# jseppanen/azalea

Hardware: AMD Instinct MI355X
Metric: mcts_sims_per_sec (higher is better)
Workload: dtype f16x3 (fp32 operands split hi+lo f16, fp32 accumulate)

## Files before the change

### azalea_amd/_lib.py

```python
import ctypes as C
import logging
import os
import subprocess

_HERE = os.path.dirname(os.path.abspath(__file__))
LIB_PATH = os.path.join(_HERE, "libazx_hip.so")

MAX_BOARD = 13
CELL_STRIDE = 192
MAX_BATCH = 16
ROW_METRICS = 8


def record_bytes(cells):
    return (16 + 5 * cells + 15) // 16 * 16

EVAL_RESNET, EVAL_UNIFORM, EVAL_UNIFORM_HASH, EVAL_EXTERNAL = 0, 1, 2, 3
FLAG_NO_COMPACT = 1
FLAG_RANDOM_REFLECT = 2
FLAG_TOWER_F16 = 4
EEXTERNAL = -7


class AzxError(RuntimeError):
# ... 74 lines not shown
    "azx_replay_state": (C.c_int, [_vp, _i64p, _i64p, _i64p]),
    "azx_replay_set_state": (C.c_int, [_vp, C.c_int64, C.c_int64]),
    "azx_replay_put": (C.c_int, [_vp, C.c_int64, _i32p, _i32p, _i32p, _f32p, _f32p]),
    "azx_replay_fill": (C.c_int, [_vp, C.c_int64, C.c_int64, _i64p, C.POINTER(PlayStats)]),
    "azx_play_device": (C.c_int, [_vp, C.c_int64, C.c_int64, _i64p, C.POINTER(PlayStats)]),
    "azx_rows_pack": (C.c_int, [_vp, C.c_int64, C.c_int64, _vp]),
    "azx_replay_put_records": (C.c_int, [_vp, C.c_int64, _vp]),
    "azx_replay_put_records_async": (C.c_int, [_vp, C.c_int64, _vp, _vp]),
    "azx_reserve_cus": (C.c_int, [_vp, C.c_int, C.POINTER(C.c_int)]),
    "azx_replay_collate": (C.c_int, [_vp, C.c_int64, _i64p, _vp, _vp, _vp, _vp, _vp, _vp, _i32p]),
    "azx_replay_collate_async": (C.c_int, [_vp, C.c_int64, _i64p, _vp, _vp, _vp, _vp, _vp, _vp, _vp]),
    "azx_replay_set_mover_view": (C.c_int, [_vp, C.c_int]),
    "azx_replay_set_reflect": (C.c_int, [_vp, C.c_int, C.c_uint64]),
    "azx_selftest_arith": (C.c_int, [C.c_int, C.c_int, _f32p, _f32p, _f32p, _f32p, _f32p]),
    "azx_selftest_divide": (C.c_int, [C.c_int, C.c_int, _f32p, _f32p, _f32p, _f32p]),
    "azx_selftest_dirichlet": (C.c_int, [C.c_int, C.c_double, C.c_int, C.c_int, C.c_uint32, _f32p]),
    "azx_debug_choose": (C.c_int, [_vp, _i32p, _f32p]),
    "azx_debug_counters": (C.c_int, [_vp, _u64p]),
    "azx_debug_counters_raw": (C.c_int, [_vp, _u64p, C.c_int64]),
    "azx_kernel_info": (C.c_int, [_vp, C.c_char_p, C.c_int]),
    "azx_debug_set_queue_cap": (C.c_int, [_vp, C.c_int64]),
    "azx_debug_stagger": (C.c_int, [_vp, _i32p]),
    "azx_debug_tower_tiles": (C.c_int, [C.c_int, C.c_char_p, C.POINTER(C.c_uint8), C.POINTER(C.c_uint32), _i32p]),
    "azx_stream": (_vp, [_vp]),
    "azx_set_external_evaluator": (C.c_int, [_vp, _vp, _vp]),
    "azx_match_create": (C.c_int, [_vp, _vp, C.POINTER(_vp)]),
    "azx_match_destroy": (None, [_vp]),
    "azx_match_play": (C.c_int, [_vp, C.c_int64, C.c_int64, C.POINTER(C.c_int8), C.POINTER(C.c_int16),
                                 C.POINTER(C.c_int16), C.POINTER(MatchStats)]),
    "azx_tournament_create": (C.c_int, [C.POINTER(_vp), C.c_int, C.POINTER(_vp)]),
    "azx_tournament_destroy": (None, [_vp]),
    "azx_tournament_play": (C.c_int, [_vp, C.c_int, _i32p, _i32p, C.c_int64, C.c_int64, C.c_int32,
                                      C.POINTER(C.c_int8), C.POINTER(C.c_int16), C.POINTER(C.c_int16),
                                      C.POINTER(MatchStats)]),
    "azx_match_set_harvest": (C.c_int, [_vp, C.c_int]),
    "azx_match_set_first_mover": (C.c_int, [_vp, C.c_int]),
    "azx_match_rows": (C.c_int, [_vp, _i64p]),
    "azx_tournament_set_harvest": (C.c_int, [_vp, C.c_int]),
    "azx_tournament_set_first_mover": (C.c_int, [_vp, C.c_int]),
    "azx_tournament_rows": (C.c_int, [_vp, _i64p]),
    "azx_rows_read": (C.c_int, [_vp, C.c_int64, C.c_int64, _i32p, _i32p, _i32p, _f32p, _f32p, _i64p]),
    "azx_openings_check": (C.c_int, [C.c_int, C.c_int, C.c_int, C.POINTER(C.c_int16), _i32p, _i32p, _i32p]),
    "azx_match_set_openings": (C.c_int, [_vp, C.c_int, C.c_int, C.POINTER(C.c_int16), _i32p]),
    "azx_tournament_set_openings": (C.c_int, [_vp, C.c_int, C.c_int, C.POINTER(C.c_int16), _i32p]),
    "azx_set_playout_cap": (C.c_int, [_vp, C.c_double, C.c_int]),
    "azx_playout_cap_is_full": (C.c_int, [C.c_uint64, C.c_int64, C.c_int, C.c_double]),
# ... 72 lines not shown
```

### azalea_amd/csrc/azx_capi.cpp

```cpp
#include <hip/hip_runtime.h>

#include <algorithm>
#include <cmath>
#include <cstdarg>
#include <cstdio>
#include <cstdlib>
#include <cstring>
#include <map>
#include <mutex>
#include <string>
#include <vector>

#include "../../include/azx.h"
#include "azx_dev.h"
#include "mcts_kernels.h"
#include "net.h"
#include "train.h"
#include "replay_kernels.h"
#include "ext_kernels.h"
#include "match_kernels.h"
#include "playout_cap.h"
#include "resign.h"
#include "tower_tiles.h"

// ... 221 lines not shown
    d.noise_alpha = (float)cfg->noise_alpha;
    d.noise_scale = 0.0;
    d.exploration_depth = cfg->exploration_depth;
    d.temperature = (float)cfg->temperature;
    e->num_batches = cfg->simulations / cfg->search_batch_size + 1;
    e->selects_per_search = e->num_batches * cfg->search_batch_size;
    d.selects_per_search = e->selects_per_search;
    int cap = cfg->nodes_per_game;
    if (cap <= 0) cap = 6 * (e->selects_per_search + 1) * d.ncells + 1024;
    d.cap = cap;

    const size_t G = d.G, bs = d.bs, E = G * bs;
    const size_t pstride = d.ncells + (d.ncells & 1);
    int rc = AZX_OK;
#define A(ptr, count) if (!rc) rc = dev_alloc(e, &ptr, (count))
    A(d.cells, G * d.slots * 64);
    A(d.ghdr, G);
    A(d.thdr, G);
    if (!rc) rc = dev_alloc(e, &d.arena[0], G * (size_t)cap, false);
    if (cfg->flags & AZX_FLAG_NO_COMPACT) d.arena[1] = d.arena[0];
    else if (!rc) rc = dev_alloc(e, &d.arena[1], G * (size_t)cap, false);
    A(d.leaf_node, E); A(d.leaf_len, E); A(d.leaf_eval, E); A(d.leaf_link, E); A(d.leaf_cells, E);
    A(d.leaf_mask, E * 4); A(d.path, E * pstride);
    A(d.ev_board, E * AZX_CELL_STRIDE); A(d.ev_src, E); A(d.ev_flip, E);
    A(d.ev_value, E); A(d.ev_prior, E * AZX_CELL_STRIDE); A(d.n_eval, 4);
    A(d.counters, G * CTR_COUNT); A(d.q_count, 2); A(d.stat_sums, G * 8);
    A(d.resign_ctr, G * RS_COUNT);
    A(d.estop_ctr, G * ES_COUNT);
    A(d.tt_ctr, G * TT_COUNT);
    A(e->g_k, G); A(e->g_legal, G * d.ncells); A(e->g_nn, G);
    A(e->g_cv, G * d.ncells); A(e->g_cw, G * d.ncells); A(e->g_cp, G * d.ncells);
    A(e->g_rv, G); A(e->g_rw, G); A(e->g_sv, G);
    A(e->moveids_dev, G); A(e->slots_dev, G); A(e->nmoves_dev, G);
#undef A
    if (rc) { azx_destroy(e); return rc; }
    if (cfg->evaluator == AZX_EVAL_RESNET) {
        rc = azx_net_create(&e->net, d.N, cfg->num_blocks, cfg->base_chans, (int)E,
                            (cfg->flags & AZX_FLAG_TOWER_F16) ? 1 : 0, e->stream);
        if (rc) { g_err = azx_net_error(); azx_destroy(e); return rc; }
    }
    {
        float *gt = nullptr;
        rc = dev_alloc(e, &gt, AZX_GAMMA_TAB_FLOATS);
        if (rc) { azx_destroy(e); return rc; }
        std::vector<float> tab(AZX_GAMMA_TAB_FLOATS, 0.0f);
        if (cfg->noise_alpha > 0.0) azx_gamma_table(cfg->noise_alpha, tab.data());
        if (hipMemcpyAsync(gt, tab.data(), tab.size() * sizeof(float), hipMemcpyHostToDevice, e->stream) != hipSuccess ||
// ... 184 lines not shown
    return (int)text.size();
}

extern "C" int azx_debug_stagger(azx_engine *e, int32_t *out4) {
    if (!e || !out4) return fail(AZX_EINVAL, "null argument");
    ENGINE_GUARD(e);
    memset(out4, 0, 4 * sizeof(int32_t));
    if (!e->stagger_ctr) return AZX_OK;
    HIPCHECK(hipMemcpyAsync(out4, e->stagger_ctr, 4 * sizeof(int32_t), hipMemcpyDeviceToHost, e->stream));
    HIPCHECK(hipStreamSynchronize(e->stream));
    return AZX_OK;
}

extern "C" int azx_debug_tower_tiles(int board_size, const char *map, uint8_t *rows256, uint32_t *skip4, int32_t *light_slot) {
    if (!map || !rows256 || !skip4 || !light_slot) return fail(AZX_EINVAL, "null argument");
    if (board_size < 2 || board_size * board_size > 121)
        return fail(AZX_EINVAL, "tower tiles: board size %d outside the fused tower's 2..11", board_size);
    if (strcmp(map, "edge") && strcmp(map, "rows")) return fail(AZX_EINVAL, "tower tiles: map '%s' is neither edge nor rows", map);
    AzxTowerTiles t;
    azx_tower_tiles_build(board_size, !strcmp(map, "edge"), &t);
    memcpy(rows256, t.row, sizeof t.row);
    for (int w = 0; w < 4; ++w) skip4[w] = t.skip[w];
    *light_slot = AZX_TOWER_LIGHT_SLOT;
    return t.edge;
}

extern "C" int azx_debug_set_queue_cap(azx_engine *e, int64_t rows) {
    if (!e || rows < 0) return fail(AZX_EINVAL, "bad argument");
    e->dbg_qcap = rows;
    return AZX_OK;
}

static int check_net_range(azx_engine *e) {
    if (!e->net) return AZX_OK;
    int rc = azx_net_check_range(e->net, e->stream);
    if (rc) g_err = azx_net_error();
    return rc;
}

extern "C" int azx_debug_weights(azx_engine *e, int which, void *out, int64_t cap, int64_t *nbytes, char *name, int name_cap) {
    if (!e) return fail(AZX_EINVAL, "null engine");
    ENGINE_GUARD(e);
    if (!e->net) return fail(AZX_ESTATE, "engine was not created with AZX_EVAL_RESNET");
    int rc = azx_net_debug_weights(e->net, which, out, cap, nbytes, name, name_cap);
    if (rc) g_err = azx_net_error();
    return rc;
// ... 2279 lines not shown
```

### azalea_amd/csrc/net.h

```cpp
#pragma once
#include <hip/hip_runtime.h>
#include <stdint.h>

#include "azx_dev.h"

struct AzxNet;

int azx_net_create(AzxNet **out, int N, int blocks, int chans, int max_evals, int tower_f16, hipStream_t st);
bool azx_net_has_fused_tower(int N, int blocks, int chans);
bool azx_net_has_f16_tower(int N, int blocks, int chans);
void azx_net_destroy(AzxNet *net);
void azx_net_set_stream(AzxNet *net, hipStream_t st, const uint32_t *mask, int words);
const char *azx_net_error();
int azx_net_set_weights(AzxNet *net, int n, const char *const *names, const void *const *ptrs,
                        const int64_t *counts, int on_device);
bool azx_net_ready(const AzxNet *net);
int azx_net_check_range(AzxNet *net, hipStream_t st);
int azx_net_debug_weights(AzxNet *net, int which, void *out, int64_t cap, int64_t *nbytes, char *name, int name_cap);
const char *azx_net_kernel_info(const AzxNet *net);
void azx_net_eval(AzxNet *net, const DevEngine &d, hipStream_t st);
bool azx_net_rows_splittable(const AzxNet *net);
void azx_net_eval_rows(AzxNet *net, const DevEngine &d, int row0, int max_n, hipStream_t st);
constexpr int AZX_NET_ROW_ALIGN = 16;
void azx_net_eval_rows_behind(AzxNet *net, const DevEngine &d, int row0, int first, int max_n, int32_t *ctr, hipStream_t st);
int azx_net_forward_host(AzxNet *net, int B, int K, const int32_t *boards,
                         const int32_t *legal_moves, float *value, float *logprob, hipStream_t st);

int azx_net_wide_train_conv(int N, int C, const unsigned short *w16, const unsigned short *in, float *out32, int n_boards,
                            const float *unscale, float2 *stat, hipStream_t st);
int azx_net_wide_train_conv_bwd(int N, int C, const unsigned short *w16, const unsigned short *in, float *g_out, int n_boards,
                                const float *unscale, float2 *pgsum, const unsigned char *mask, const float *raw, const float *skip,
                                const double *sums, float invN, unsigned int *gmax, hipStream_t st);
```

### azalea_amd/csrc/net_kernels.hip

```cpp
#include "net_priv.h"
#include "tower_tiles.h"

#ifndef AZX_NET_ABLATE
#define AZX_NET_ABLATE 0
#endif
#ifndef AZX_SAT_TRACK
#define AZX_SAT_TRACK 1
#endif

#include <cmath>
#include <cstdio>
#include <cstdlib>
#include <cstring>
#include <map>
#include <string>
#include <type_traits>
#include <utility>
#include <vector>

typedef float f32x16 __attribute__((ext_vector_type(16)));

static thread_local std::string g_net_err;
const char *azx_net_error() { return g_net_err.c_str(); }

// ... 168 lines not shown
#define WT_FLUSH if (lane == 0) { for (int r_ = 0; r_ < 7; ++r_) atomicAdd(&g_wide_stamp[r_], nt_acc[r_]); atomicAdd(&g_wide_stamp[7], 1ull); \
    atomicAdd(&g_wide_stamp[8], __builtin_amdgcn_s_memrealtime() - nt_rt0); }
#else
#define NT_DECL
#define NT_MARK(r)
#define NT_FLUSH
#define WT_FLUSH
#endif

#ifndef F16X3_BPB
#define F16X3_BPB 2
#endif
#ifndef AZX_S16_FENCE
#define AZX_S16_FENCE 1
#endif
typedef float f32x4 __attribute__((ext_vector_type(4)));

__global__ __launch_bounds__(F16X3_BPB * 128, 2) void k_tower_f16x3_s16(NetDev P, const uint8_t *__restrict__ ev_board,
                                                                        const int32_t *__restrict__ n_eval_ptr,
                                                                        int n_eval_host, float *__restrict__ act_out,
                                                                        float *__restrict__ hfeat) {
    constexpr int C = 64, ROWB = 272, MT = 4, NT = 4;
    extern __shared__ __align__(16) unsigned char smem[];
    const int n_eval = n_eval_ptr ? *n_eval_ptr : n_eval_host;
    const int e0 = blockIdx.x * F16X3_BPB;
    if (e0 >= n_eval) return;
    const int tid = threadIdx.x, lane = tid & 63, wave = __builtin_amdgcn_readfirstlane(tid >> 6);
    NT_DECL
    const int wb = wave >> 1, wh = wave & 1;
    const int N = P.N, ncells = P.ncells;
    const int e = e0 + wb;
    const bool live = e < n_eval;
    const int board_b = 128 * ROWB;
    const int zero_off = 0;
    const int x_off = 2 * ROWB + wb * board_b;
    unsigned char *X = smem + x_off;
    const int li = lane & 15, lh = lane >> 4;
    const int lrow = li < 8 ? li ^ 4 : li;
    const int lchunk = 128 * (lh & 1) + 16 * (lh >> 1);

    constexpr int LT = AZX_TOWER_LIGHT_SLOT;
    static_assert(LT == MT - 1, "the k-loop skips the lagging last tile");
    const uint8_t *tmap = P.tile_map + 64 * wave + lrow;
    const uint32_t skip = __builtin_amdgcn_readfirstlane((uint32_t)(P.tile_skip >> (9 * wave)) & 0x1ffu);
    unsigned long long tapok = 0ull;
    int rbase[MT], cell0_[MT];
#pragma unroll
    for (int m = 0; m < MT; ++m) {
        const int L = tmap[16 * m];
        const int r = L & 127;
        const int ry = r / N, rx = r - ry * N;
        cell0_[m] = r < ncells ? 2 * ROWB + (L >> 7) * board_b + 121 * ROWB + ry * (N + 2) + rx : -1;
        rbase[m] = 2 * ROWB + L * ROWB + lchunk;
#pragma unroll
        for (int tap = 0; tap < 9; ++tap) {
            const int yy = ry + tap / 3 - 1, xx = rx + tap % 3 - 1;
            if (r < ncells && yy >= 0 && yy < N && xx >= 0 && xx < N) tapok |= 1ull << (tap * 4 + m);
        }
    }
    uint32_t tapok_lo = (uint32_t)tapok, tapok_hi = (uint32_t)(tapok >> 32);
    auto act_offset = [&](int tap, int m) -> int {
        const int delta = ((tap / 3 - 1) * N + (tap % 3 - 1)) * ROWB;
        const uint32_t word = tap < 8 ? tapok_lo : tapok_hi;
        const int mask = (int)(word << (31 - ((tap * 4 + m) & 31))) >> 31;
        return (mask | 0xF0) & (rbase[m] + delta);
    };

    f32x4 res[MT][NT];
    auto load_bias = [&](const float *bias, float4 (&b4)[NT]) {
#pragma unroll
        for (int n = 0; n < NT; ++n) b4[n] = *reinterpret_cast<const float4 *>(bias + 16 * n + 4 * lh);
    };
    float satmax = 0.f;
    auto epilogue = [&](f32x4 (&acc)[MT][NT], const float4 (&bias4)[NT], auto kind_tag) {
        constexpr int kind = decltype(kind_tag)::value;
#pragma unroll
        for (int n = 0; n < NT; ++n) {
            const float4 b4 = bias4[n];
            const float bv[4] = {b4.x, b4.y, b4.z, b4.w};
#pragma unroll
            for (int m = 0; m < MT; ++m) {
                float v4[4];
#pragma unroll
                for (int j = 0; j < 4; ++j) {
                    float v = acc[m][n][j] + bv[j];
                    if (kind == 1) v += res[m][n][j];
                    v = fmaxf(v, 0.0f);
                    if (kind != 0) res[m][n][j] = v;
                    v4[j] = v;
                }
                if (AZX_SAT_TRACK) {
                    satmax = fmaxf(fmaxf(satmax, v4[0]), fmaxf(v4[1], fmaxf(v4[2], v4[3])));
                    asm volatile("" : "+v"(satmax));
                }
                uint2 h4, l4;
                split2_f16(v4[0], v4[1], h4.x, l4.x);
                split2_f16(v4[2], v4[3], h4.y, l4.y);
                unsigned char *pw = smem + rbase[m] + (112 * (lh >> 1) - 120 * (lh & 1)) + 16 * n;
                *reinterpret_cast<uint2 *>(pw) = h4;
                *reinterpret_cast<uint2 *>(pw + 64) = l4;
            }
        }
    };

    {
        const int NH = N + 2;
        unsigned char *cells = X + 121 * ROWB;
        const uint8_t *bd = ev_board + (size_t)(live ? e : n_eval - 1) * AZX_CELL_STRIDE;
        if (wh == 0) {
            for (int i = lane; i < NH * NH; i += 64) {
                const int y = i / NH - 1, x = i - (y + 1) * NH - 1;
                cells[i] = (y >= 0 && y < N && x >= 0 && x < N) ? bd[y * N + x] : (uint8_t)3;
            }
        }
        for (int i = tid; i < 2 * ROWB / 4; i += F16X3_BPB * 128) reinterpret_cast<uint32_t *>(smem + zero_off)[i] = 0u;
        __syncthreads();
        f32x4 acc[MT][NT];
#pragma unroll
        for (int m = 0; m < MT; ++m)
#pragma unroll
            for (int n = 0; n < NT; ++n) acc[m][n] = f32x4{0.f, 0.f, 0.f, 0.f};
        const uint4 *ws = reinterpret_cast<const uint4 *>(P.Ws16);
        f16x8 wfh[NT], wfl[NT];
#pragma unroll
        for (int n = 0; n < NT; ++n) {
            const uint4 qh = ws[(n * 2) * 64 + lane], ql = ws[(n * 2 + 1) * 64 + lane];
            wfh[n] = *reinterpret_cast<const f16x8 *>(&qh);
            wfl[n] = *reinterpret_cast<const f16x8 *>(&ql);
        }
#pragma unroll
        for (int m = 0; m < MT; ++m) {
            uint32_t onehot = 0u;
            if (cell0_[m] >= 0) {
                const unsigned char *c0 = smem + cell0_[m];
#pragma unroll
                for (int tap = 0; tap < 9; ++tap) {
                    const uint32_t v = c0[(tap / 3) * NH + tap % 3];
                    onehot |= (v < 3u ? 1u : 0u) << (3 * tap + v);
                }
            }
            const uint32_t byte = (onehot >> (8 * lh)) & 0xffu;
            uint4 q;
            q.x = ((byte >> 0) & 1u) * 0x3C00u | ((byte >> 1) & 1u) * 0x3C000000u;
            q.y = ((byte >> 2) & 1u) * 0x3C00u | ((byte >> 3) & 1u) * 0x3C000000u;
            q.z = ((byte >> 4) & 1u) * 0x3C00u | ((byte >> 5) & 1u) * 0x3C000000u;
            q.w = ((byte >> 6) & 1u) * 0x3C00u | ((byte >> 7) & 1u) * 0x3C000000u;
            const f16x8 xf = *reinterpret_cast<const f16x8 *>(&q);
#pragma unroll
            for (int n = 0; n < NT; ++n) {
                acc[m][n] = __builtin_amdgcn_mfma_f32_16x16x32_f16(wfh[n], xf, acc[m][n], 0, 0, 0);
                acc[m][n] = __builtin_amdgcn_mfma_f32_16x16x32_f16(wfl[n], xf, acc[m][n], 0, 0, 0);
            }
        }
        float4 sb4[NT];
        load_bias(P.stem_b, sb4);
        __syncthreads();
        epilogue(acc, sb4, std::integral_constant<int, 2>{});
    }
    __syncthreads();
    NT_MARK(0)

    const uint4 *wsrc = reinterpret_cast<const uint4 *>(P.Wh16);
    int stage = 0;
    const int last_stage = P.layers * 18 - 1;
    f16x8 wh_[NT], wl_[NT];
    auto load_w = [&](int st, int nn, int part) {
        const uint4 qq = wsrc[(size_t)min(st, last_stage) * 512 + (nn * 2 + part) * 64 + lane];
        if (part) wl_[nn] = *reinterpret_cast<const f16x8 *>(&qq);
        else wh_[nn] = *reinterpret_cast<const f16x8 *>(&qq);
    };
#pragma unroll
    for (int i = 0; i < 4; ++i) load_w(0, i >> 1, i & 1);
    auto conv_layer = [&](int layer, auto residual_tag) {
        constexpr bool residual = decltype(residual_tag)::value;
        asm volatile("" : "+v"(tapok_lo), "+v"(tapok_hi), "+v"(rbase[0]), "+v"(rbase[1]), "+v"(rbase[2]), "+v"(rbase[3]));
        f32x4 acc[MT][NT];
#pragma unroll
        for (int m = 0; m < MT; ++m)
// ... 1445 lines not shown
    bool want_edge = true;
    { const char *v = getenv("AZX_TOWER_TILES"); want_edge = !(v && !strcmp(v, "rows")); }
    azx_tower_tiles_build(N, x3 && want_edge, &tiles);
    {
        char b[320];
        const char *tower = "k_stem_generic + k_conv_generic (VALU)";
        if (net->tower_variant == 4) tower = net->tower_f16 ? "k_tower_f16_s16" : "k_tower_f16x3_s16";
        else if (net->tower_variant == 5) tower = net->tower_f16 ? "k_stem_wide_f16 + k_conv_wide_f16_s16 per layer"
                                                                 : "k_stem_wide_f16x3 + k_conv_wide_f16x3_s16 per layer";
        else if (net->tower_variant == 1) tower = "k_tower_mfma<64,4,2,1,2> (fp32 MFMA)";
        else if (net->tower_variant == 2) tower = "k_tower_mfma<64,6,1,2,2> (fp32 MFMA)";
        else if (net->tower_variant == 3) tower = "k_tower_mfma<32,6,2,2,1> (fp32 MFMA)";
        const bool hm = net->tower_variant == 4 && net->opt_heads_mfma && ncells <= 128;
        snprintf(b, sizeof b, "%s + %s (%dx%d on %dx%d; AZX_TOWER=%s AZX_TOWER_TILES=%s AZX_WIDE_STREAMS=%d AZX_HEADS=%s AZX_PACK=%s)",
                 tower, hm ? "k_heads_mfma" : "k_heads", blocks, chans, N, N, want_fp32 ? "fp32" : net->tower_f16 ? "f16" : "default",
                 want_edge && (tiles.edge || !x3) ? "edge" : "rows",
                 net->opt_wsplit, net->opt_heads_mfma ? "mfma" : "valu", net->pack_on_host ? "host" : "device");
        net->info = b;
    }
    const size_t E = max_evals;
    net->act = nalloc<float>(net, E * ncells * chans);
    net->logit = nalloc<float>(net, E * AZX_CELL_STRIDE);
    if (net->tower_variant == 4) net->hfeat = nalloc<float>(net, E * 6 * ncells);
    net->hb_board = nalloc<uint8_t>(net, E * AZX_CELL_STRIDE);
    net->hb_flip = nalloc<int32_t>(net, E);
    net->hb_value = nalloc<float>(net, E);
    if (!net->use_mfma) {
        net->act2 = nalloc<float>(net, E * ncells * chans);
        net->act3 = nalloc<float>(net, E * ncells * chans);
    }
    if (net->tower_variant == 5) {
        net->wideX = nalloc<unsigned short>(net, E * ncells * chans * 2);
        net->wideY = nalloc<unsigned short>(net, E * ncells * chans * 2);
    }
    if (!net->act || !net->logit || !net->hb_board || !net->hb_flip || !net->hb_value ||
        (!net->use_mfma && (!net->act2 || !net->act3)) || (net->tower_variant == 5 && (!net->wideX || !net->wideY))) {
        azx_net_destroy(net);
        return nfail(AZX_ENOMEM, "net: hipMalloc failed");
    }
    const int bpb = net->tower_variant == 2 ? 1 : 2;
    net->lds_bytes = (size_t)bpb * 2 * (ncells + 1) * (chans + 4) * sizeof(float);
    if (net->tower_variant == 4) net->lds_bytes = (size_t)F16X3_BPB * 128 * 272 + 2 * 272;
    if (net->tower_variant == 5) net->lds_bytes = (size_t)(ncells + 2) * WIDE_ROWB;
    net->d.sat_flag = nalloc<uint32_t>(net, 4);
    if (x3) {
        uint8_t *tm = nalloc<uint8_t>(net, sizeof tiles.row);
        if (tm && hipMemcpy(tm, tiles.row, sizeof tiles.row, hipMemcpyHostToDevice) != hipSuccess) tm = nullptr;
        if (!tm) {
            azx_net_destroy(net);
            return nfail(AZX_ENOMEM, "net: the tower's tile map could not be put on the device");
        }
        net->d.tile_map = tm;
        for (int w = 0; w < 4; ++w) net->d.tile_skip |= (unsigned long long)(tiles.skip[w] & 0x1ffu) << (9 * w);
    }
    if (!net->d.sat_flag || hipDeviceSynchronize() != hipSuccess) {
        azx_net_destroy(net);
        return nfail(AZX_ENOMEM, "net: hipMalloc failed");
    }
    *out = net;
    return AZX_OK;
}

void azx_net_set_stream(AzxNet *net, hipStream_t st, const uint32_t *mask, int words) {
    if (!net) return;
    for (int i = 0; i < 3; ++i) {
        if (net->stream2[i]) { (void)hipStreamSynchronize(net->stream2[i]); (void)hipStreamDestroy(net->stream2[i]); }
        if (net->ev_join[i]) (void)hipEventDestroy(net->ev_join[i]);
        net->stream2[i] = nullptr;
        net->ev_join[i] = nullptr;
    }
    if (net->ev_fork) (void)hipEventDestroy(net->ev_fork);
    net->ev_fork = nullptr;
    net->streams_ok = false;
    net->cu_mask.assign(mask, mask + (mask ? words : 0));
    net->stream = st;
// ... 32 lines not shown
            static const char *nm[7] = {"stem", "residual load/setup", "k-loop (MFMA)", "barrier after k-loop",
                                        "epilogue", "barrier after epilogue", "output store"};
            unsigned long long tot = 0;
            for (int r = 0; r < 7; ++r) tot += h[r];
            fprintf(stderr, "k_tower_f16x3_s16 stamps over %llu blocks: %.0f cycles/block, shader clock %.0f MHz during the kernel\n",
                    h[7], (double)tot / h[7], h[8] ? 100.0 * (double)tot / (double)h[8] : 0.0);
            for (int r = 0; r < 7; ++r)
                fprintf(stderr, "  %-24s %6.1f%%  %9.0f cycles/block\n", nm[r], 100.0 * h[r] / tot, (double)h[r] / h[7]);
            {
                std::vector<unsigned long long> tr(3 * 32768);
                (void)hipMemcpyFromSymbol(tr.data(), HIP_SYMBOL(g_tower_trace), tr.size() * sizeof(unsigned long long));
                std::map<unsigned long long, std::vector<std::pair<unsigned long long, unsigned long long>>> cu;
                unsigned long long t0 = ~0ull, t1 = 0;
                size_t nblk = 0;
                for (int b = 0; b < 32768; ++b)
                    if (tr[3 * b + 2]) {
                        cu[tr[3 * b]].push_back({tr[3 * b + 1], tr[3 * b + 2]});
                        t0 = std::min(t0, tr[3 * b + 1]);
                        t1 = std::max(t1, tr[3 * b + 2]);
                        ++nblk;
                    }
                double busy = 0, mn = 1e30, mx = 0, lastend_min = 1e30, lastend_max = 0;
                size_t cmin = 1 << 30, cmax = 0;
                for (auto &kv : cu) {
                    double b = 0, le = 0;
                    for (auto &iv : kv.second) { b += (double)(iv.second - iv.first); le = std::max(le, (double)(iv.second - t0)); }
                    busy += b; mn = std::min(mn, b); mx = std::max(mx, b);
                    cmin = std::min(cmin, kv.second.size()); cmax = std::max(cmax, kv.second.size());
                    lastend_min = std::min(lastend_min, le); lastend_max = std::max(lastend_max, le);
                }
                fprintf(stderr, "  last launch: %zu blocks on %zu CUs, span %.1f us, blocks/CU %zu..%zu, mean resident blocks/CU %.2f, "
                        "per-CU block-time %.0f..%.0f us, CU finish %.0f..%.0f us\n", nblk, cu.size(), (t1 - t0) / 100.0, cmin, cmax,
                        busy / ((double)(t1 - t0) * cu.size()), mn / 100.0, mx / 100.0, lastend_min / 100.0, lastend_max / 100.0);
            }
            int nb = -1;
            (void)hipOccupancyMaxActiveBlocksPerMultiprocessor(&nb, (const void *)k_tower_f16x3_s16, F16X3_BPB * 128, net->lds_bytes);
            hipFuncAttributes fa;
            memset(&fa, 0, sizeof fa);
            (void)hipFuncGetAttributes(&fa, (const void *)k_tower_f16x3_s16);
            fprintf(stderr, "  runtime occupancy: %d blocks/CU (dynamic LDS %zu B, static %zu B, %d VGPRs, max threads %d)\n", nb,
                    net->lds_bytes, (size_t)fa.sharedSizeBytes, fa.numRegs, fa.maxThreadsPerBlock);
        }
    }
#endif
    if (!net) return;
    for (void *p : net->allocs) (void)hipFree(p);
    if (net->raw_tab_host) (void)hipHostFree((void *)net->raw_tab_host);
    if (net->wmax_host) (void)hipHostFree((void *)net->wmax_host);
    delete net;
}

bool azx_net_ready(const AzxNet *net) { return net && net->ready; }


static void run_net(AzxNet *net, const uint8_t *boards, const int32_t *flip, const int32_t *n_eval_ptr,
                    int n_host, int max_n, float *logit, float *value, float *prior, hipStream_t st, size_t row0 = 0) {
    const NetDev &d = net->d;
    if (max_n <= 0) return;
    const size_t act_rows = row0 * d.ncells * d.C;
    float *const act = net->act + act_rows;
    float *const act2 = net->act2 ? net->act2 + act_rows : nullptr;
    float *const act3 = net->act3 ? net->act3 + act_rows : nullptr;
    float *const hfeat_rows = net->hfeat ? net->hfeat + row0 * 6 * d.ncells : nullptr;
    const float *hfeat = nullptr;
    if (net->use_mfma) {
        const size_t lds = net->lds_bytes;
        if (net->tower_variant == 4) {
            const dim3 grid((max_n + F16X3_BPB - 1) / F16X3_BPB), block(F16X3_BPB * 128);
            if (net->tower_f16) hipLaunchKernelGGL(k_tower_f16_s16, grid, block, lds, st, d, boards, n_eval_ptr, n_host, hfeat_rows);
            else hipLaunchKernelGGL(k_tower_f16x3_s16, grid, block, lds, st, d, boards, n_eval_ptr, n_host, (float *)nullptr, hfeat_rows);
            hfeat = hfeat_rows;
        } else if (net->tower_variant == 5) {
            const dim3 grid(max_n, d.C / 128), block(256);
            const auto k_stem = net->tower_f16 ? k_stem_wide_f16 : k_stem_wide_f16x3;
            const auto k_conv = net->tower_f16 ? k_conv_wide_f16_s16 : k_conv_wide_f16x3_s16;
            hipLaunchKernelGGL(k_stem, grid, block, 0, st, d, boards, net->wideX,
                               d.blocks == 0 ? net->act : (float *)nullptr, n_eval_ptr, n_host);
            const int wsplit = net->opt_wsplit;
            {
                int parts = wsplit;
                if (parts > 1 && !net->ev_fork) {
                    bool ok = hipEventCreateWithFlags(&net->ev_fork, hipEventDisableTiming) == hipSuccess;
                    for (int i = 0; i < 3 && ok; ++i)
                        ok = (net->cu_mask.empty() ? hipStreamCreateWithFlags(&net->stream2[i], hipStreamNonBlocking)
                                                   : hipExtStreamCreateWithCUMask(&net->stream2[i], (uint32_t)net->cu_mask.size(), net->cu_mask.data())) == hipSuccess &&
                             hipEventCreateWithFlags(&net->ev_join[i], hipEventDisableTiming) == hipSuccess;
                    net->streams_ok = ok;
                }
                if (parts > 1 && !net->streams_ok) parts = 1;
                const int per = (((max_n + parts - 1) / parts + 7) / 8) * 8;
                if (per >= max_n) parts = 1;
// ... 43 lines not shown
        hipLaunchKernelGGL(k_heads_mfma, dim3((max_n + HM_MB - 1) / HM_MB), dim3(256), hl, st, d, hfeat, boards, flip, n_eval_ptr, n_host, logit, value, prior);
    } else {
        const size_t hl = ((size_t)(6 * d.ncells + 64) * HEADS_BPB + (size_t)HEADS_BPB * AZX_CELL_STRIDE +
                           (size_t)(HEADS_KSPLIT - 1) * (64 + 192) * HEADS_BPB) * sizeof(float);
        hipLaunchKernelGGL(k_heads, dim3((max_n + HEADS_BPB - 1) / HEADS_BPB), dim3(192 * HEADS_KSPLIT), hl, st, d, act, hfeat, boards, flip, n_eval_ptr, n_host, logit, value, prior);
    }
}

const char *azx_net_kernel_info(const AzxNet *net) { return net->info.c_str(); }

int azx_net_check_range(AzxNet *net, hipStream_t st) {
    if (!net || !net->d.sat_flag) return AZX_OK;
    uint32_t flag = 0;
    if (hipMemcpyAsync(&flag, net->d.sat_flag, sizeof flag, hipMemcpyDeviceToHost, st) != hipSuccess ||
        hipStreamSynchronize(st) != hipSuccess)
        return nfail(AZX_EHIP, "net: reading the activation range flag failed");
    if (!flag) return AZX_OK;
    (void)hipMemsetAsync(net->d.sat_flag, 0, sizeof flag, st);
    return nfail(AZX_ERANGE, "net: an activation of the residual tower exceeded the f16 range (65504) of the f16 tower "
                             "kernels (split-f16 and plain f16 alike) -- the evaluations of this call are not valid (AZX_TOWER=fp32 runs the fp32 MFMA tower)");
}

void azx_net_eval(AzxNet *net, const DevEngine &e, hipStream_t st) {
    run_net(net, e.ev_board, e.ev_flip, e.n_eval, 0, net->max_evals, net->logit, e.ev_value, e.ev_prior, st);
}

bool azx_net_rows_splittable(const AzxNet *net) { return net && !(net->use_mfma && net->tower_variant == 5); }

void azx_net_eval_rows(AzxNet *net, const DevEngine &e, int row0, int max_n, hipStream_t st) {
    run_net(net, e.ev_board, e.ev_flip, e.n_eval, 0, max_n, net->logit + (size_t)row0 * AZX_CELL_STRIDE, e.ev_value,
            e.ev_prior, st, (size_t)row0);
}

__global__ void k_rows_behind(const int32_t *__restrict__ n_eval_ptr, int first, int32_t *__restrict__ ctr) {
    if (threadIdx.x != 0 || blockIdx.x != 0) return;
    const int n = *n_eval_ptr;
    const int rest = n > first ? n - first : 0;
    ctr[0] = rest;
    ctr[1] = n;
    ctr[2] = ctr[2] + 1;
    ctr[3] = ctr[3] + (rest == 0 ? 1 : 0);
}

static_assert(AZX_NET_ROW_ALIGN % HM_MB == 0 && AZX_NET_ROW_ALIGN % HEADS_BPB == 0 && AZX_NET_ROW_ALIGN % F16X3_BPB == 0 &&
              AZX_NET_ROW_ALIGN % 2 == 0, "AZX_NET_ROW_ALIGN: whole blocks of k_tower_f16x3_s16, k_tower_mfma (1 or 2 boards), k_heads_mfma, k_heads");
void azx_net_eval_rows_behind(AzxNet *net, const DevEngine &e, int row0, int first, int max_n, int32_t *ctr, hipStream_t st) {
    if (first <= 0 || first >= max_n) return;
    hipLaunchKernelGGL(k_rows_behind, dim3(1), dim3(64), 0, st, (const int32_t *)e.n_eval, first, ctr);
    const size_t f = (size_t)first;
    run_net(net, e.ev_board + f * AZX_CELL_STRIDE, e.ev_flip + f, ctr, 0, max_n - first,
            net->logit + ((size_t)row0 + f) * AZX_CELL_STRIDE, e.ev_value + f, e.ev_prior + f * AZX_CELL_STRIDE, st,
            (size_t)row0 + f);
}

int azx_net_forward_host(AzxNet *net, int B, int K, const int32_t *boards, const int32_t *legal_moves,
                         float *value, float *logprob, hipStream_t st) {
    if (!net->ready) return nfail(AZX_ESTATE, "net: azx_set_weights has not been called");
    if (B < 0 || K < 0 || (B && (!boards || !legal_moves || !value || !logprob)))
        return nfail(AZX_EINVAL, "net: bad forward arguments");
    const NetDev &d = net->d;
    const int ncells = d.ncells;
    std::vector<uint8_t> hb((size_t)net->max_evals * AZX_CELL_STRIDE);
    std::vector<float> hl((size_t)net->max_evals * AZX_CELL_STRIDE), hv(net->max_evals);
    for (int b0 = 0; b0 < B; b0 += net->max_evals) {
        const int nb = std::min(net->max_evals, B - b0);
        std::fill(hb.begin(), hb.end(), 0);
        for (int i = 0; i < nb; ++i)
            for (int c = 0; c < ncells; ++c) {
                const int32_t v = boards[(size_t)(b0 + i) * ncells + c];
                if (v < 0 || v > 2) return nfail(AZX_EINVAL, "net: board values must be 0/1/2");
                hb[(size_t)i * AZX_CELL_STRIDE + c] = (uint8_t)v;
            }
        if (hipMemcpyAsync(net->hb_board, hb.data(), (size_t)nb * AZX_CELL_STRIDE, hipMemcpyHostToDevice, st) != hipSuccess)
            return nfail(AZX_EHIP, "net: H2D copy failed");
        run_net(net, net->hb_board, net->hb_flip, nullptr, nb, nb, net->logit, net->hb_value, nullptr, st);
        if (hipGetLastError() != hipSuccess) return nfail(AZX_EHIP, "net: kernel launch failed");
        if (hipMemcpyAsync(hl.data(), net->logit, (size_t)nb * AZX_CELL_STRIDE * sizeof(float), hipMemcpyDeviceToHost, st) != hipSuccess ||
            hipMemcpyAsync(hv.data(), net->hb_value, (size_t)nb * sizeof(float), hipMemcpyDeviceToHost, st) != hipSuccess ||
            hipStreamSynchronize(st) != hipSuccess)
            return nfail(AZX_EHIP, "net: D2H copy failed");
        for (int i = 0; i < nb; ++i) {
            value[b0 + i] = hv[i];
            const int32_t *lm = legal_moves + (size_t)(b0 + i) * K;
            float *lp = logprob + (size_t)(b0 + i) * K;
            float mx = -INFINITY;
            for (int j = 0; j < K; ++j) {
                if (lm[j] < 0 || lm[j] > ncells) return nfail(AZX_EINVAL, "net: legal move out of range");
                const int tile = lm[j] > 0 ? lm[j] - 1 : 0;
                lp[j] = lm[j] == 0 ? -99.0f : hl[(size_t)i * AZX_CELL_STRIDE + tile];
                mx = std::max(mx, lp[j]);
            }
            double sum = 0.0;
            for (int j = 0; j < K; ++j) sum += std::exp((double)lp[j] - (double)mx);
            const float lse = (float)((double)mx + std::log(sum));
            for (int j = 0; j < K; ++j) lp[j] = lp[j] - lse;
        }
    }
    return AZX_OK;
// ... 2 lines not shown
```

### azalea_amd/csrc/net_priv.h

```cpp
#pragma once
#include <hip/hip_runtime.h>
#include <stdint.h>

#include <algorithm>
#include <string>
#include <vector>

#include "net.h"

struct NetDev {
    int N, ncells, C, blocks, layers;
    const float *stemT;
    const float *stem_b;
    const unsigned short *Ws;
    const unsigned short *Ws16, *Wh16;
    const unsigned short *Whd16;
    const float *hbias16;
    const float *Wp;
    const float *Wg;
    const float *bias;
    const float *wv, *bv;
    const float *wp, *bp;
    const float *fc2T, *fc2b;
    const float *fc3w, *fc3b;
    const float *mfcT, *mfcb;
    const float *hmP, *hmV;
    int hm_lda;
    uint32_t *sat_flag;
    const uint8_t *tile_map;
    unsigned long long tile_skip;
};

#ifndef AZX_LO_BITS
#define AZX_LO_BITS 10
#endif
#define LO_MASK ((0xFFFFu << (10 - AZX_LO_BITS)) & 0xFFFFu)
#define LO_RND (AZX_LO_BITS < 10 ? (1u << (9 - AZX_LO_BITS)) : 0u)
static inline unsigned short lo_round_bits(unsigned short bits) {
    return (unsigned short)((bits + LO_RND) & LO_MASK);
}

struct AzxNet {
    NetDev d;
    int max_evals = 0;
    bool ready = false;
    bool use_mfma = false;
    hipStream_t stream = nullptr;
    std::vector<void *> allocs;
    float *act = nullptr, *act2 = nullptr, *act3 = nullptr;
    unsigned short *wideX = nullptr, *wideY = nullptr;
    float *logit = nullptr;
    float *hfeat = nullptr;
    uint8_t *hb_board = nullptr;
// ... 37 lines not shown
```

### azalea_amd/csrc/tower_tiles.h

```cpp
#pragma once
#include <stdint.h>

#define AZX_TOWER_LIGHT_SLOT 3

struct AzxTowerTiles {
    uint8_t row[256];
    uint32_t skip[4];
    int edge;
};

static inline bool azx_tile_tap_is_padding(int N, int L, int tap) {
    const int cell = L & 127;
    if (cell >= N * N) return true;
    const int y = cell / N + tap / 3 - 1, x = cell % N + tap % 3 - 1;
    return y < 0 || y >= N || x < 0 || x >= N;
}

static inline void azx_tower_tiles_rows(AzxTowerTiles *t) {
    for (int i = 0; i < 256; ++i) t->row[i] = (uint8_t)i;
    for (int w = 0; w < 4; ++w) t->skip[w] = 0u;
    t->edge = 0;
}

static inline void azx_tile_slot_keys(int L, int tile_row, int *k1, int *k2) {
    const bool a = (tile_row & 4) == 0;
    *k1 = (L + (a ? 8 : 0)) & 15;
    *k2 = (L + (a ? 0 : 8)) & 15;
}

static inline void azx_tower_tiles_build(int N, int edge, AzxTowerTiles *t) {
    azx_tower_tiles_rows(t);
    if (!edge || N < 2 || N * N > 121) return;
    const int ncells = N * N;
    int cls[256];
    for (int L = 0; L < 256; ++L) {
        const int cell = L & 127, y = cell / N, x = cell % N;
        cls[L] = cell >= ncells ? 5 : y == 0 ? 0 : y == N - 1 ? 1 : x == 0 ? 2 : x == N - 1 ? 3 : 4;
    }
    bool used[256] = {false};
    int light[4][16];
    for (int c = 0; c < 4; ++c) {
        int nres[16] = {0}, chosen[16];
        for (int k = 0; k < 16; ++k) {
            int best = -1;
            for (int pass = 0; pass < 2 && best < 0; ++pass)
                for (int L = 0; L < 256; ++L)
                    if (!used[L] && cls[L] == (pass ? 5 : c) && (best < 0 || nres[L & 15] < nres[best & 15])) best = L;
            if (best < 0) { azx_tower_tiles_rows(t); return; }
            used[best] = true;
            ++nres[best & 15];
            chosen[k] = best;
        }
        int n1[16] = {0}, n2[16] = {0};
// ... 38 lines not shown
```

### include/azx.h

```cpp
#ifndef AZX_H
#define AZX_H

#include <stdint.h>

#ifdef __cplusplus
extern "C" {
#endif

#define AZX_MAX_BOARD 13
#define AZX_MAX_CELLS (AZX_MAX_BOARD * AZX_MAX_BOARD)
#define AZX_CELL_STRIDE 192
#define AZX_MAX_BATCH 16
#define AZX_ROW_METRICS 8
#define AZX_RECORD_BYTES(cells) ((size_t)((16 + 5 * (cells) + 15) / 16 * 16))

enum {
    AZX_OK = 0,
    AZX_EINVAL = -1,
    AZX_EHIP = -2,
    AZX_ENOMEM = -3,
    AZX_ESTATE = -4,
    AZX_ENODEV = -5,
    AZX_ERANGE = -6,
    AZX_EEXTERNAL = -7
// ... 163 lines not shown
#define AZX_ROWS_REFERENCE 0
#define AZX_ROWS_VISITS    1
int azx_set_train_targets(azx_engine *e, int policy_rows, float value_mix);
int azx_get_train_targets(azx_engine *e, int *policy_rows, float *value_mix);
int azx_train_targets_stats(azx_engine *e, int64_t out4[4]);

int azx_selftest_arith(int device, int n, const float *a, const float *b, float *sq, float *dv,
                       float *mul);

int azx_selftest_divide(int device, int n, const float *num, const float *den, float *quot,
                        float *sqrt_tab);

int azx_selftest_dirichlet(int device, double alpha, int k, int n_rows, uint32_t seed, float *out);

int azx_debug_choose(azx_engine *e, int32_t *move_id, float *moves_prob);

int azx_debug_counters(azx_engine *e, uint64_t *out16);
int azx_debug_counters_raw(azx_engine *e, uint64_t *out, int64_t n_games);

int azx_kernel_info(azx_engine *e, char *buf, int cap);
int azx_debug_set_queue_cap(azx_engine *e, int64_t rows);
int azx_debug_stagger(azx_engine *e, int32_t *out4);
int azx_debug_tower_tiles(int board_size, const char *map, uint8_t *rows256, uint32_t *skip4, int32_t *light_slot);

typedef struct {
    int64_t games;
    int64_t wins[2];
    int64_t first_player_wins;
    int64_t voided;
    int64_t plies;
    double  seconds;
} azx_match_stats;
typedef struct azx_match azx_match;
int azx_match_create(azx_engine *a, azx_engine *b, azx_match **out);
void azx_match_destroy(azx_match *m);
int azx_match_play(azx_match *m, int64_t first_game, int64_t n_games, int8_t *outcome, int16_t *length,
                   int16_t *moves, azx_match_stats *stats);

int azx_match_set_harvest(azx_match *m, int on);
int azx_match_set_first_mover(azx_match *m, int mode);
int azx_match_rows(azx_match *m, int64_t *rows_out);

typedef struct azx_tournament azx_tournament;
int azx_tournament_create(azx_engine *const *engines, int n_engines, azx_tournament **out);
void azx_tournament_destroy(azx_tournament *t);
int azx_tournament_play(azx_tournament *t, int n_pairs, const int32_t *pair_a, const int32_t *pair_b,
// ... 34 lines not shown
```

Measured before the change: 5.505 million.

## Precompute per-lane tile words and hoist tower prologue loads before n_eval check

Moves the stem's per-lane tile geometry (row, cell offset, tap validity, dead flag) into a host-built 32-bit lane table, so the kernel reads one word per tile instead of doing divides and a 9-tap loop. Board bytes, stem weights and biases are issued before the dependent n_eval read and pinned in registers, so their latency overlaps the n_eval fetch. The board buffer gains one slack row so blocks can read past the live rows without faulting, with an abort guard on launch. It also adds a debug export of the lane table and a CU gap statistic in the profiling path.

```diff
diff --git a/azalea_amd/_lib.py b/azalea_amd/_lib.py
--- a/azalea_amd/_lib.py
+++ b/azalea_amd/_lib.py
@@ -120,6 +120,7 @@
     "azx_debug_set_queue_cap": (C.c_int, [_vp, C.c_int64]),
     "azx_debug_stagger": (C.c_int, [_vp, _i32p]),
     "azx_debug_tower_tiles": (C.c_int, [C.c_int, C.c_char_p, C.POINTER(C.c_uint8), C.POINTER(C.c_uint32), _i32p]),
+    "azx_debug_tower_lanes": (C.c_int, [C.c_int, C.c_char_p, C.POINTER(C.c_uint32)]),
     "azx_stream": (_vp, [_vp]),
     "azx_set_external_evaluator": (C.c_int, [_vp, _vp, _vp]),
     "azx_match_create": (C.c_int, [_vp, _vp, C.POINTER(_vp)]),
diff --git a/azalea_amd/csrc/azx_capi.cpp b/azalea_amd/csrc/azx_capi.cpp
--- a/azalea_amd/csrc/azx_capi.cpp
+++ b/azalea_amd/csrc/azx_capi.cpp
@@ -267,7 +267,7 @@
     else if (!rc) rc = dev_alloc(e, &d.arena[1], G * (size_t)cap, false);
     A(d.leaf_node, E); A(d.leaf_len, E); A(d.leaf_eval, E); A(d.leaf_link, E); A(d.leaf_cells, E);
     A(d.leaf_mask, E * 4); A(d.path, E * pstride);
-    A(d.ev_board, E * AZX_CELL_STRIDE); A(d.ev_src, E); A(d.ev_flip, E);
+    A(d.ev_board, (E + AZX_NET_BOARD_SLACK) * AZX_CELL_STRIDE); A(d.ev_src, E); A(d.ev_flip, E);
     A(d.ev_value, E); A(d.ev_prior, E * AZX_CELL_STRIDE); A(d.n_eval, 4);
     A(d.counters, G * CTR_COUNT); A(d.q_count, 2); A(d.stat_sums, G * 8);
     A(d.resign_ctr, G * RS_COUNT);
@@ -498,6 +498,17 @@
     memcpy(rows256, t.row, sizeof t.row);
     for (int w = 0; w < 4; ++w) skip4[w] = t.skip[w];
     *light_slot = AZX_TOWER_LIGHT_SLOT;
+    return t.edge;
+}
+
+extern "C" int azx_debug_tower_lanes(int board_size, const char *map, uint32_t *words256) {
+    if (!map || !words256) return fail(AZX_EINVAL, "null argument");
+    if (board_size < 2 || board_size * board_size > 121)
+        return fail(AZX_EINVAL, "tower lanes: board size %d outside the fused tower's 2..11", board_size);
+    if (strcmp(map, "edge") && strcmp(map, "rows")) return fail(AZX_EINVAL, "tower lanes: map '%s' is neither edge nor rows", map);
+    AzxTowerTiles t;
+    azx_tower_tiles_build(board_size, !strcmp(map, "edge"), &t);
+    memcpy(words256, t.lane, sizeof t.lane);
     return t.edge;
 }
 
diff --git a/azalea_amd/csrc/net.h b/azalea_amd/csrc/net.h
--- a/azalea_amd/csrc/net.h
+++ b/azalea_amd/csrc/net.h
@@ -18,6 +18,7 @@
 int azx_net_check_range(AzxNet *net, hipStream_t st);
 int azx_net_debug_weights(AzxNet *net, int which, void *out, int64_t cap, int64_t *nbytes, char *name, int name_cap);
 const char *azx_net_kernel_info(const AzxNet *net);
+constexpr int AZX_NET_BOARD_SLACK = 1;
 void azx_net_eval(AzxNet *net, const DevEngine &d, hipStream_t st);
 bool azx_net_rows_splittable(const AzxNet *net);
 void azx_net_eval_rows(AzxNet *net, const DevEngine &d, int row0, int max_n, hipStream_t st);
diff --git a/azalea_amd/csrc/net_kernels.hip b/azalea_amd/csrc/net_kernels.hip
--- a/azalea_amd/csrc/net_kernels.hip
+++ b/azalea_amd/csrc/net_kernels.hip
@@ -214,47 +214,82 @@
                                                                         float *__restrict__ hfeat) {
     constexpr int C = 64, ROWB = 272, MT = 4, NT = 4;
     extern __shared__ __align__(16) unsigned char smem[];
-    const int n_eval = n_eval_ptr ? *n_eval_ptr : n_eval_host;
-    const int e0 = blockIdx.x * F16X3_BPB;
-    if (e0 >= n_eval) return;
     const int tid = threadIdx.x, lane = tid & 63, wave = __builtin_amdgcn_readfirstlane(tid >> 6);
     NT_DECL
+    const int e0 = blockIdx.x * F16X3_BPB;
     const int wb = wave >> 1, wh = wave & 1;
     const int N = P.N, ncells = P.ncells;
     const int e = e0 + wb;
+    const int li = lane & 15, lh = lane >> 4;
+    const int lrow = li < 8 ? li ^ 4 : li;
+
+    const int n_eval = n_eval_ptr ? *n_eval_ptr : n_eval_host;
+    constexpr int LT = AZX_TOWER_LIGHT_SLOT;
+    const uint32_t *ltab = P.lane_tab + 64 * wave + lrow;
+    uint32_t lw[MT];
+#pragma unroll
+    for (int m = 0; m < MT; ++m) lw[m] = ltab[16 * m];
+    const int NH = N + 2;
+    const uint32_t nh_magic = 65536u / (uint32_t)NH + 1u;
+    int cidx[3];
+    uint32_t cbyte[3];
+    {
+        const uint8_t *bd = ev_board + (size_t)e * AZX_CELL_STRIDE;
+#pragma unroll
+        for (int k = 0; k < 3; ++k) {
+            const int i = lane + 64 * k;
+            const int yq = (int)(((uint32_t)i * nh_magic) >> 16), y = yq - 1, x = i - yq * NH - 1;
+            const bool on = ((uint32_t)y < (uint32_t)N) & ((uint32_t)x < (uint32_t)N);
+            cidx[k] = on ? y * N + x : -1;
+            cbyte[k] = 3u;
+        }
+        if (wh == 0) {
+#pragma unroll
+            for (int k = 0; k < 3; ++k) cbyte[k] = bd[max(cidx[k], 0)];
+        }
+    }
+    f16x8 wfh[NT], wfl[NT];
+    {
+        const f16x8 *ws = reinterpret_cast<const f16x8 *>(P.Ws16);
+#pragma unroll
+        for (int n = 0; n < NT; ++n) {
+            wfh[n] = ws[(n * 2) * 64 + lane];
+            wfl[n] = ws[(n * 2 + 1) * 64 + lane];
+        }
+    }
+    f32x4 sbv[NT];
+#pragma unroll
+    for (int n = 0; n < NT; ++n) sbv[n] = *reinterpret_cast<const f32x4 *>(P.stem_b + 16 * n + 4 * lh);
+    asm volatile("" : "+v"(lw[0]), "+v"(lw[1]), "+v"(lw[2]), "+v"(lw[3]), "+v"(cbyte[0]), "+v"(cbyte[1]), "+v"(cbyte[2]),
+                      "+v"(wfh[0]), "+v"(wfh[1]), "+v"(wfh[2]), "+v"(wfh[3]), "+v"(wfl[0]), "+v"(wfl[1]), "+v"(wfl[2]), "+v"(wfl[3]),
+                      "+v"(sbv[0]), "+v"(sbv[1]), "+v"(sbv[2]), "+v"(sbv[3]));
+    if (e0 >= n_eval) return;
     const bool live = e < n_eval;
     const int board_b = 128 * ROWB;
     const int zero_off = 0;
     const int x_off = 2 * ROWB + wb * board_b;
     unsigned char *X = smem + x_off;
-    const int li = lane & 15, lh = lane >> 4;
-    const int lrow = li < 8 ? li ^ 4 : li;
     const int lchunk = 128 * (lh & 1) + 16 * (lh >> 1);
 
-    constexpr int LT = AZX_TOWER_LIGHT_SLOT;
     static_assert(LT == MT - 1, "the k-loop skips the lagging last tile");
     const uint8_t *tmap = P.tile_map + 64 * wave + lrow;
     const uint32_t skip = __builtin_amdgcn_readfirstlane((uint32_t)(P.tile_skip >> (9 * wave)) & 0x1ffu);
-    unsigned long long tapok = 0ull;
     int rbase[MT], cell0_[MT];
+    uint32_t dead = 0u;
 #pragma unroll
     for (int m = 0; m < MT; ++m) {
-        const int L = tmap[16 * m];
-        const int r = L & 127;
-        const int ry = r / N, rx = r - ry * N;
-        cell0_[m] = r < ncells ? 2 * ROWB + (L >> 7) * board_b + 121 * ROWB + ry * (N + 2) + rx : -1;
+        const int L = (lw[m] >> AZX_LANE_ROW_SHIFT) & 0xff;
+        cell0_[m] = 2 * ROWB + (L >> 7) * board_b + 121 * ROWB + (int)((lw[m] >> AZX_LANE_CELL0_SHIFT) & 0xff);
         rbase[m] = 2 * ROWB + L * ROWB + lchunk;
-#pragma unroll
-        for (int tap = 0; tap < 9; ++tap) {
-            const int yy = ry + tap / 3 - 1, xx = rx + tap % 3 - 1;
-            if (r < ncells && yy >= 0 && yy < N && xx >= 0 && xx < N) tapok |= 1ull << (tap * 4 + m);
-        }
-    }
-    uint32_t tapok_lo = (uint32_t)tapok, tapok_hi = (uint32_t)(tapok >> 32);
+        dead |= ((lw[m] >> AZX_LANE_DEAD_BIT) & 1u) << m;
+    }
+    static_assert(MT == 4, "tapok: tiles 0..2 in the low word, tile 3 in the high one");
+    uint32_t tapok_lo = AZX_LANE_TAPS(lw[0]) | (AZX_LANE_TAPS(lw[1]) << 9) | (AZX_LANE_TAPS(lw[2]) << 18);
+    uint32_t tapok_hi = AZX_LANE_TAPS(lw[3]);
     auto act_offset = [&](int tap, int m) -> int {
         const int delta = ((tap / 3 - 1) * N + (tap % 3 - 1)) * ROWB;
-        const uint32_t word = tap < 8 ? tapok_lo : tapok_hi;
-        const int mask = (int)(word << (31 - ((tap * 4 + m) & 31))) >> 31;
+        const uint32_t word = m < 3 ? tapok_lo : tapok_hi;
+        const int mask = (int)(word << (31 - (9 * (m % 3) + tap))) >> 31;
         return (mask | 0xF0) & (rbase[m] + delta);
     };
 
@@ -296,13 +331,17 @@
     };
 
     {
-        const int NH = N + 2;
         unsigned char *cells = X + 121 * ROWB;
-        const uint8_t *bd = ev_board + (size_t)(live ? e : n_eval - 1) * AZX_CELL_STRIDE;
         if (wh == 0) {
-            for (int i = lane; i < NH * NH; i += 64) {
-                const int y = i / NH - 1, x = i - (y + 1) * NH - 1;
-                cells[i] = (y >= 0 && y < N && x >= 0 && x < N) ? bd[y * N + x] : (uint8_t)3;
+            if (!live) {
+                const uint8_t *bd = ev_board + (size_t)(n_eval - 1) * AZX_CELL_STRIDE;
+#pragma unroll
+                for (int k = 0; k < 3; ++k) cbyte[k] = bd[max(cidx[k], 0)];
+            }
+#pragma unroll
+            for (int k = 0; k < 3; ++k) {
+                const int i = lane + 64 * k;
+                if (i < NH * NH) cells[i] = (uint8_t)(cidx[k] >= 0 ? cbyte[k] : 3u);
             }
         }
         for (int i = tid; i < 2 * ROWB / 4; i += F16X3_BPB * 128) reinterpret_cast<uint32_t *>(smem + zero_off)[i] = 0u;
@@ -312,25 +351,19 @@
         for (int m = 0; m < MT; ++m)
 #pragma unroll
             for (int n = 0; n < NT; ++n) acc[m][n] = f32x4{0.f, 0.f, 0.f, 0.f};
-        const uint4 *ws = reinterpret_cast<const uint4 *>(P.Ws16);
-        f16x8 wfh[NT], wfl[NT];
-#pragma unroll
-        for (int n = 0; n < NT; ++n) {
-            const uint4 qh = ws[(n * 2) * 64 + lane], ql = ws[(n * 2 + 1) * 64 + lane];
-            wfh[n] = *reinterpret_cast<const f16x8 *>(&qh);
-            wfl[n] = *reinterpret_cast<const f16x8 *>(&ql);
-        }
 #pragma unroll
         for (int m = 0; m < MT; ++m) {
             uint32_t onehot = 0u;
-            if (cell0_[m] >= 0) {
-                const unsigned char *c0 = smem + cell0_[m];
-#pragma unroll
-                for (int tap = 0; tap < 9; ++tap) {
-                    const uint32_t v = c0[(tap / 3) * NH + tap % 3];
-                    onehot |= (v < 3u ? 1u : 0u) << (3 * tap + v);
-                }
-            }
+#pragma unroll
+            for (int ty = 0; ty < 3; ++ty) {
+                const int a = cell0_[m] + ty * NH;
+#pragma unroll
+                for (int tx = 0; tx < 3; ++tx) {
+                    const uint32_t v = smem[a + tx];
+                    onehot |= (v < 3u ? 1u : 0u) << (3 * (3 * ty + tx) + v);
+                }
+            }
+            if ((dead >> m) & 1u) onehot = 0u;
             const uint32_t byte = (onehot >> (8 * lh)) & 0xffu;
             uint4 q;
             q.x = ((byte >> 0) & 1u) * 0x3C00u | ((byte >> 1) & 1u) * 0x3C000000u;
@@ -345,7 +378,8 @@
             }
         }
         float4 sb4[NT];
-        load_bias(P.stem_b, sb4);
+#pragma unroll
+        for (int n = 0; n < NT; ++n) sb4[n] = make_float4(sbv[n][0], sbv[n][1], sbv[n][2], sbv[n][3]);
         __syncthreads();
         epilogue(acc, sb4, std::integral_constant<int, 2>{});
     }
@@ -1837,7 +1871,7 @@
     net->act = nalloc<float>(net, E * ncells * chans);
     net->logit = nalloc<float>(net, E * AZX_CELL_STRIDE);
     if (net->tower_variant == 4) net->hfeat = nalloc<float>(net, E * 6 * ncells);
-    net->hb_board = nalloc<uint8_t>(net, E * AZX_CELL_STRIDE);
+    net->hb_board = nalloc<uint8_t>(net, (E + AZX_NET_BOARD_SLACK) * AZX_CELL_STRIDE);
     net->hb_flip = nalloc<int32_t>(net, E);
     net->hb_value = nalloc<float>(net, E);
     if (!net->use_mfma) {
@@ -1861,11 +1895,14 @@
     if (x3) {
         uint8_t *tm = nalloc<uint8_t>(net, sizeof tiles.row);
         if (tm && hipMemcpy(tm, tiles.row, sizeof tiles.row, hipMemcpyHostToDevice) != hipSuccess) tm = nullptr;
-        if (!tm) {
+        uint32_t *lt = nalloc<uint32_t>(net, 256);
+        if (lt && hipMemcpy(lt, tiles.lane, sizeof tiles.lane, hipMemcpyHostToDevice) != hipSuccess) lt = nullptr;
+        if (!tm || !lt) {
             azx_net_destroy(net);
             return nfail(AZX_ENOMEM, "net: the tower's tile map could not be put on the device");
         }
         net->d.tile_map = tm;
+        net->d.lane_tab = lt;
         for (int w = 0; w < 4; ++w) net->d.tile_skip |= (unsigned long long)(tiles.skip[w] & 0x1ffu) << (9 * w);
     }
     if (!net->d.sat_flag || hipDeviceSynchronize() != hipSuccess) {
@@ -1944,6 +1981,23 @@
                     }
                 double busy = 0, mn = 1e30, mx = 0, lastend_min = 1e30, lastend_max = 0;
                 size_t cmin = 1 << 30, cmax = 0;
+                double gap = 0;
+                size_t ngap = 0;
+                for (auto &kv : cu) {
+                    std::vector<unsigned long long> ss, ee;
+                    for (auto &iv : kv.second) { ss.push_back(iv.first); ee.push_back(iv.second); }
+                    std::sort(ss.begin(), ss.end());
+                    std::sort(ee.begin(), ee.end());
+                    size_t j = 0;
+                    for (unsigned long long en : ee) {
+                        while (j < ss.size() && ss[j] < en) ++j;
+                        if (j == ss.size()) break;
+                        gap += (double)(ss[j++] - en);
+                        ++ngap;
+                    }
+                }
+                fprintf(stderr, "  last launch: mean gap from a block's end to the next block's start on its CU %.2f us (%zu pairs, 10 ns ticks)\n",
+                        ngap ? gap / ngap / 100.0 : 0.0, ngap);
                 for (auto &kv : cu) {
                     double b = 0, le = 0;
                     for (auto &iv : kv.second) { b += (double)(iv.second - iv.first); le = std::max(le, (double)(iv.second - t0)); }
@@ -1975,7 +2029,7 @@
 bool azx_net_ready(const AzxNet *net) { return net && net->ready; }
 
 
-static void run_net(AzxNet *net, const uint8_t *boards, const int32_t *flip, const int32_t *n_eval_ptr,
+static void run_net(AzxNet *net, const uint8_t *boards, size_t board_rows, const int32_t *flip, const int32_t *n_eval_ptr,
                     int n_host, int max_n, float *logit, float *value, float *prior, hipStream_t st, size_t row0 = 0) {
     const NetDev &d = net->d;
     if (max_n <= 0) return;
@@ -1989,6 +2043,10 @@
         const size_t lds = net->lds_bytes;
         if (net->tower_variant == 4) {
             const dim3 grid((max_n + F16X3_BPB - 1) / F16X3_BPB), block(F16X3_BPB * 128);
+            if ((size_t)grid.x * F16X3_BPB > board_rows) {
+                fprintf(stderr, "net: a tower launch of %d rows (%u blocks) reaches past the %zu board rows behind it\n", max_n, grid.x, board_rows);
+                abort();
+            }
             if (net->tower_f16) hipLaunchKernelGGL(k_tower_f16_s16, grid, block, lds, st, d, boards, n_eval_ptr, n_host, hfeat_rows);
             else hipLaunchKernelGGL(k_tower_f16x3_s16, grid, block, lds, st, d, boards, n_eval_ptr, n_host, (float *)nullptr, hfeat_rows);
             hfeat = hfeat_rows;
@@ -2078,13 +2136,14 @@
 }
 
 void azx_net_eval(AzxNet *net, const DevEngine &e, hipStream_t st) {
-    run_net(net, e.ev_board, e.ev_flip, e.n_eval, 0, net->max_evals, net->logit, e.ev_value, e.ev_prior, st);
+    run_net(net, e.ev_board, (size_t)net->max_evals + AZX_NET_BOARD_SLACK, e.ev_flip, e.n_eval, 0, net->max_evals, net->logit, e.ev_value,
+            e.ev_prior, st);
 }
 
 bool azx_net_rows_splittable(const AzxNet *net) { return net && !(net->use_mfma && net->tower_variant == 5); }
 
 void azx_net_eval_rows(AzxNet *net, const DevEngine &e, int row0, int max_n, hipStream_t st) {
-    run_net(net, e.ev_board, e.ev_flip, e.n_eval, 0, max_n, net->logit + (size_t)row0 * AZX_CELL_STRIDE, e.ev_value,
+    run_net(net, e.ev_board, (size_t)net->max_evals + AZX_NET_BOARD_SLACK - (size_t)row0, e.ev_flip, e.n_eval, 0, max_n, net->logit + (size_t)row0 * AZX_CELL_STRIDE, e.ev_value,
             e.ev_prior, st, (size_t)row0);
 }
 
@@ -2104,7 +2163,8 @@
     if (first <= 0 || first >= max_n) return;
     hipLaunchKernelGGL(k_rows_behind, dim3(1), dim3(64), 0, st, (const int32_t *)e.n_eval, first, ctr);
     const size_t f = (size_t)first;
-    run_net(net, e.ev_board + f * AZX_CELL_STRIDE, e.ev_flip + f, ctr, 0, max_n - first,
+    run_net(net, e.ev_board + f * AZX_CELL_STRIDE, (size_t)net->max_evals + AZX_NET_BOARD_SLACK - (size_t)row0 - f, e.ev_flip + f, ctr, 0,
+            max_n - first,
             net->logit + ((size_t)row0 + f) * AZX_CELL_STRIDE, e.ev_value + f, e.ev_prior + f * AZX_CELL_STRIDE, st,
             (size_t)row0 + f);
 }
@@ -2129,7 +2189,8 @@
             }
         if (hipMemcpyAsync(net->hb_board, hb.data(), (size_t)nb * AZX_CELL_STRIDE, hipMemcpyHostToDevice, st) != hipSuccess)
             return nfail(AZX_EHIP, "net: H2D copy failed");
-        run_net(net, net->hb_board, net->hb_flip, nullptr, nb, nb, net->logit, net->hb_value, nullptr, st);
+        run_net(net, net->hb_board, (size_t)net->max_evals + AZX_NET_BOARD_SLACK, net->hb_flip, nullptr, nb, nb, net->logit, net->hb_value,
+                nullptr, st);
         if (hipGetLastError() != hipSuccess) return nfail(AZX_EHIP, "net: kernel launch failed");
         if (hipMemcpyAsync(hl.data(), net->logit, (size_t)nb * AZX_CELL_STRIDE * sizeof(float), hipMemcpyDeviceToHost, st) != hipSuccess ||
             hipMemcpyAsync(hv.data(), net->hb_value, (size_t)nb * sizeof(float), hipMemcpyDeviceToHost, st) != hipSuccess ||
diff --git a/azalea_amd/csrc/net_priv.h b/azalea_amd/csrc/net_priv.h
--- a/azalea_amd/csrc/net_priv.h
+++ b/azalea_amd/csrc/net_priv.h
@@ -29,6 +29,7 @@
     uint32_t *sat_flag;
     const uint8_t *tile_map;
     unsigned long long tile_skip;
+    const uint32_t *lane_tab;
 };
 
 #ifndef AZX_LO_BITS
diff --git a/azalea_amd/csrc/tower_tiles.h b/azalea_amd/csrc/tower_tiles.h
--- a/azalea_amd/csrc/tower_tiles.h
+++ b/azalea_amd/csrc/tower_tiles.h
@@ -3,10 +3,16 @@
 
 #define AZX_TOWER_LIGHT_SLOT 3
 
+#define AZX_LANE_TAPS(w) ((w) & 0x1ffu)
+#define AZX_LANE_CELL0_SHIFT 9
+#define AZX_LANE_ROW_SHIFT 17
+#define AZX_LANE_DEAD_BIT 25
+
 struct AzxTowerTiles {
     uint8_t row[256];
     uint32_t skip[4];
     int edge;
+    uint32_t lane[256];
 };
 
 static inline bool azx_tile_tap_is_padding(int N, int L, int tap) {
@@ -28,7 +34,29 @@
     *k2 = (L + (a ? 0 : 8)) & 15;
 }
 
+static inline void azx_tower_tiles_lanes(int N, AzxTowerTiles *t) {
+    for (int i = 0; i < 256; ++i) {
+        const int L = t->row[i], cell = L & 127;
+        uint32_t w = (uint32_t)L << AZX_LANE_ROW_SHIFT;
+        if (N < 1 || cell >= N * N) {
+            w |= 1u << AZX_LANE_DEAD_BIT;
+        } else {
+            for (int tap = 0; tap < 9; ++tap)
+                if (!azx_tile_tap_is_padding(N, L, tap)) w |= 1u << tap;
+            w |= (uint32_t)((cell / N) * (N + 2) + cell % N) << AZX_LANE_CELL0_SHIFT;
+        }
+        t->lane[i] = w;
+    }
+}
+
+static inline void azx_tower_tiles_map(int N, int edge, AzxTowerTiles *t);
+
 static inline void azx_tower_tiles_build(int N, int edge, AzxTowerTiles *t) {
+    azx_tower_tiles_map(N, edge, t);
+    azx_tower_tiles_lanes(N, t);
+}
+
+static inline void azx_tower_tiles_map(int N, int edge, AzxTowerTiles *t) {
     azx_tower_tiles_rows(t);
     if (!edge || N < 2 || N * N > 121) return;
     const int ncells = N * N;
diff --git a/include/azx.h b/include/azx.h
--- a/include/azx.h
+++ b/include/azx.h
@@ -209,6 +209,7 @@
 int azx_debug_set_queue_cap(azx_engine *e, int64_t rows);
 int azx_debug_stagger(azx_engine *e, int32_t *out4);
 int azx_debug_tower_tiles(int board_size, const char *map, uint8_t *rows256, uint32_t *skip4, int32_t *light_slot);
+int azx_debug_tower_lanes(int board_size, const char *map, uint32_t *words256);
 
 typedef struct {
     int64_t games;
```

Measured after the change: 5.518 million (median of 6 runs). Within noise of the previous version (+0.2%).
